# iitmdinesh/image2text

Hardware: AMD Instinct MI355X
Metric: train images/sec + greedy captions/sec, nano config (higher is better)
Workload: dtype bf16; 1 GPU; nano-224 (6x512 ViT encoder + 12x768 nanoGPT decoder, 224x224x3 images, 64-token captions); global_batch=3072, per_gpu_batch=3072, caption_len=64, parallelism=dp1, optimizer=AdamW lr 6e-4 betas (0.9,0.95), weights=random init (reference distributions)

## Files before the change

### image2text_amd/csrc/gemm.hip

```cpp
#include "common.h"
#include <stdlib.h>
#include <string.h>
#include <utility>

namespace {

constexpr int BM = 128, BN = 128, BK = 64;
constexpr int R_ROW_BYTES = 128;
constexpr int CF_ROW_BYTES = 288;
constexpr int OPERAND_BYTES = 128 * 128;
constexpr int STAGE_BYTES = 2 * OPERAND_BYTES;
constexpr int SMEM_BYTES = 2 * STAGE_BYTES;

struct GemmParams {
    const bf16_t* A;
    const bf16_t* B;
    void* C;
    int M, N, K;
    int lda, ldb, ldc;
    float alpha;
    const float* alpha_sumsq;
    const float* bias;
    int act;
    const bf16_t* aux_in;
// ... 2 lines not shown
    int ld_aux_out;
    const float* residual;
    int ldr;
    int c_is_f32;
    int accumulate;
    int tiles_m, tiles_n;
    int drop_mode;
    unsigned drop_key, drop_thr;
    float drop_scale;
    float* ws;
    int g2_splits, g2_nk;
    int g2_gn;
    int g2_dbg;
    const float* scale_a = nullptr;
    const float* scale_b = nullptr;
    int g2_stagger, g2_stagger_groups;
    const bf16_t* xq; long xq_bs; int xq_rs;
    const int* xcu;
    bf16_t* xo; long xo_bs; int xo_rs;
    float* xlse;
    int x_total_q, x_TqMax, x_H, x_d, x_B;
};

constexpr int GN_MAX = 16;
__device__ __forceinline__ void tile_coords(const GemmParams& p, int swz, int& tile_m, int& tile_n, int gn_max = GN_MAX) {
    const int gn = p.tiles_n < gn_max ? p.tiles_n : gn_max;
    const int per_group = p.tiles_m * gn;
    int grp = swz / per_group;
    const int ngroups = (p.tiles_n + gn - 1) / gn;
    int rem = swz - grp * per_group, width = gn;
// ... 816 lines not shown

#ifndef G2_SETPRIO
#define G2_SETPRIO 0
#endif
constexpr int G2_UNIT = 128 * 128;
constexpr int G2_SMEM = 8 * G2_UNIT + 8 * 4096;
typedef __attribute__((address_space(3))) void* lds_ptr_t;

struct G2Tile {
    const bf16_t* a;
    const bf16_t* b;
    unsigned a_bytes, b_bytes;
    int m0, n0, t0;
};

template <bool A_KMAJOR, bool B_KMAJOR, bool UNSWAP = false, bool XA = false>
struct G2 {
    static constexpr bool PK = A_KMAJOR && B_KMAJOR;
    static constexpr int FA = A_KMAJOR ? 2 : 1, FB = B_KMAJOR ? 2 : 1;
    static constexpr int cap(int n) { return n > 15 ? 15 : n; }
    static constexpr int LG0 = cap(4 * FA + 4 * FB), LG1 = cap(4 * FA), LG2 = cap(4 * FA), LG3 = cap(4 * FA + 4 * FB);

    static constexpr int phys(int slot) { return ((slot & 3) == 0 || (slot & 3) == 3) ? (slot >> 2) * 2 + ((slot & 3) == 3) : 4 + (slot >> 2) * 2 + ((slot & 3) == 2); }
    unsigned char* smem;
    int lane, wr, wc, wave_off, nk, tb, ta;
    int va[2][2], vb[2][2];
    unsigned step_a, step_b;
    unsigned lds0;
    G2Tile cur, nxt;

    __device__ __forceinline__ static G2Tile tile_desc(const GemmParams& p, int idx, int ntiles) {
        G2Tile d;
        if (idx >= ntiles) {
            d.a = p.A; d.b = p.B; d.a_bytes = 0; d.b_bytes = 0; d.m0 = 0; d.n0 = 0; d.t0 = 0;
            return d;
        }
        const int tiles = p.tiles_m * p.tiles_n, slice = idx / tiles;
        d.t0 = slice * p.g2_nk;
        int tile_m, tile_n;
        tile_coords(p, idx - slice * tiles, tile_m, tile_n, p.g2_gn);
        d.m0 = tile_m * 256; d.n0 = tile_n * 256;
        if (XA) {
            d.a = p.A + (size_t)tile_m * 128 * p.lda;
            d.a_bytes = (unsigned)((p.x_d + 128) * p.lda * 2);
// ... 109 lines not shown
#pragma unroll
                for (int j = 0; j < 2; ++j) rb[ks * 2 + j] = dma_frag_read<B_KMAJOR, PK>(smem + phys(SLOT) * G2_UNIT, wc * 32 + j * 16, ks, lane);
        }
    }
    template <int SUBA, int SUBB, int KS>
    __device__ __forceinline__ void mma(f32x4 (&acc)[8][4], const bf16x8 (&ra)[8], const bf16x8 (&rb)[4]) {
        if (G2_SETPRIO) __builtin_amdgcn_s_setprio(1);
#pragma unroll
        for (int i = 0; i < 4; ++i)
#pragma unroll
            for (int j = 0; j < 2; ++j)
                acc[SUBA * 4 + i][SUBB * 2 + j] =
                    (UNSWAP || (XA && SUBA == 0)) ? __builtin_amdgcn_mfma_f32_16x16x32_bf16(ra[KS * 4 + i], rb[KS * 2 + j], acc[SUBA * 4 + i][SUBB * 2 + j], 0, 0, 0)
                           : __builtin_amdgcn_mfma_f32_16x16x32_bf16(rb[KS * 2 + j], ra[KS * 4 + i], acc[SUBA * 4 + i][SUBB * 2 + j], 0, 0, 0);
        if (G2_SETPRIO) __builtin_amdgcn_s_setprio(0);
    }
    template <int LG>
    __device__ __forceinline__ void fence() {
        asm volatile("s_waitcnt vmcnt(6) lgkmcnt(%0)" ::"n"(LG) : "memory");
        __builtin_amdgcn_s_barrier();
    }

    template <bool LAST>
    __device__ __forceinline__ void two_tiles(int t, f32x4 (&acc)[8][4], bf16x8 (&ra)[8], bf16x8 (&rb0)[4], bf16x8 (&rb1)[4]) {
        fence<LG3>();  read_a<0, 1>(ra);  read_b<2>(rb1);  stage<1, 2>(t + 1);
        mma<0, 0, 0>(acc, ra, rb0);  mma<0, 0, 1>(acc, ra, rb0);
        fence<LG0>();  stage<1, 3>(t + 1);
        mma<0, 1, 0>(acc, ra, rb1);  read_a<3, 0>(ra);  mma<0, 1, 1>(acc, ra, rb1);
        fence<LG1>();  read_a<3, 1>(ra);  stage<0, 0>(t + 2);
        mma<1, 1, 0>(acc, ra, rb1);  mma<1, 1, 1>(acc, ra, rb1);
        fence<LG2>();  read_b<5>(rb1);  stage<0, 1>(t + 2);
        mma<1, 0, 0>(acc, ra, rb0);  read_a<4, 0>(ra);  mma<1, 0, 1>(acc, ra, rb0);
        fence<LG3>();  read_a<4, 1>(ra);  read_b<6>(rb0);  stage<0, 2>(t + 2);
        mma<0, 1, 0>(acc, ra, rb1);  mma<0, 1, 1>(acc, ra, rb1);
        fence<LG0>();  stage<0, 3>(t + 2);
        mma<0, 0, 0>(acc, ra, rb0);  read_a<7, 0>(ra);  mma<0, 0, 1>(acc, ra, rb0);
        fence<LG1>();  read_a<7, 1>(ra);  stage<1, 0>(t + 3);
        mma<1, 0, 0>(acc, ra, rb0);  mma<1, 0, 1>(acc, ra, rb0);
        fence<LG2>();  if (!LAST) read_b<1>(rb0);  stage<1, 1>(t + 3);
        mma<1, 1, 0>(acc, ra, rb1);  if (!LAST) read_a<0, 0>(ra);  mma<1, 1, 1>(acc, ra, rb1);
    }
    __device__ __forceinline__ void next_tile_reads(bf16x8 (&ra)[8], bf16x8 (&rb0)[4]) {
        read_b<1>(rb0);
        read_a<0, 0>(ra);
    }

    typedef __attribute__((ext_vector_type(8))) int i32x8;
// ... 102 lines not shown
    return (const GemmParams*)k;
}

template <bool A_KMAJOR, bool B_KMAJOR, int EPI>
__global__ __launch_bounds__(512) void gemm256_kernel(GemmParams p) {
    __shared__ __attribute__((aligned(16))) unsigned char smem[G2_SMEM];
    const int tid = threadIdx.x;
    const int G = gridDim.x, bid = blockIdx.x, ntiles = p.tiles_m * p.tiles_n * p.g2_splits;
    const int xcd = bid & 7, q8 = G >> 3, r8 = G & 7;
    const int first = (xcd < r8 ? xcd * (q8 + 1) : r8 * (q8 + 1) + (xcd - r8) * q8) + (bid >> 3);

    if (p.g2_stagger > 0) {
        const int k = ((bid >> 3) % p.g2_stagger_groups) * p.g2_stagger;
        for (int i = 0; i < k; ++i) __builtin_amdgcn_s_sleep(127);
    }
    G2<A_KMAJOR, B_KMAJOR, EPI == 6, EPI == 8> g;
    g.init(p, smem, tid);
    g.cur = g.tile_desc(p, first, ntiles);
    g.nxt = g.tile_desc(p, first + G, ntiles);
    f32x4 acc[8][4];
    if constexpr (EPI == 9) {
        typename decltype(g)::i32x8 fa[4], fb0[2], fb1[2];
        g.template stage<0, 0>(0); g.template stage<0, 1>(0); g.template stage<0, 2>(0); g.template stage<0, 3>(0);
        g.template stage<1, 0>(1); g.template stage<1, 1>(1);
        asm volatile("s_waitcnt vmcnt(8)" ::: "memory");
        __builtin_amdgcn_s_barrier();
        g.next_tile_reads_fp8(fa, fb0);
        for (int idx = first; idx < ntiles; idx += G) {
#pragma unroll
            for (int i = 0; i < 8; ++i)
#pragma unroll
// ... 18 lines not shown
    }
    bf16x8 ra[8], rb0[4], rb1[4];

    g.template stage<0, 0>(0); g.template stage<0, 1>(0); g.template stage<0, 2>(0); g.template stage<0, 3>(0);
    g.template stage<1, 0>(1); g.template stage<1, 1>(1);
    asm volatile("s_waitcnt vmcnt(8)" ::: "memory");
    __builtin_amdgcn_s_barrier();
    g.template read_b<1>(rb0);
    g.template read_a<0, 0>(ra);

    for (int idx = first; idx < ntiles; idx += G) {
#pragma unroll
        for (int i = 0; i < 8; ++i)
#pragma unroll
            for (int j = 0; j < 4; ++j) acc[i][j] = f32x4{0.f, 0.f, 0.f, 0.f};
        for (int t = 0; t < g.nk - 2; t += 2) g.template two_tiles<false>(t, acc, ra, rb0, rb1);
        g.template two_tiles<true>(g.nk - 2, acc, ra, rb0, rb1);
        const int m0 = g.cur.m0, n0 = g.cur.n0;
        g.cur = g.nxt;
        g.nxt = g.tile_desc(p, idx + 2 * G, ntiles);
        if constexpr (EPI == 8) {
            int lane_e = tid & 63;
            asm volatile("" : "+v"(lane_e));
            xattn_epilogue(*epilogue_params(), acc, m0 >> 8, n0, g.wr, g.wc, lane_e, smem + 8 * G2_UNIT + (g.wave_off << 2));
        } else if constexpr (EPI == 12) {
            int lane_e = tid & 63;
            asm volatile("" : "+v"(lane_e));
            top2_epilogue(*epilogue_params(), acc, m0 + g.wr * 128, n0 + g.wc * 64, lane_e);
        } else if constexpr (EPI == 6) {
            int lane_e = tid & 63;
            asm volatile("" : "+v"(lane_e));
            float* C = reinterpret_cast<float*>(p.C);
            const float alpha = eff_alpha(p);
            const int mb = m0 + g.wr * 128 + 4 * (lane_e >> 4), n_ = n0 + g.wc * 64 + (lane_e & 15);
#pragma unroll
            for (int i = 0; i < 8; ++i)
#pragma unroll
                for (int j = 0; j < 4; ++j)
#pragma unroll
                    for (int r = 0; r < 4; ++r) {
                        const int m = mb + i * 16 + r, n = n_ + j * 16;
                        if (m < p.M && n < p.N && !(p.g2_dbg & 2)) atomicAdd(C + (size_t)m * p.ldc + n, acc[i][j][r] * alpha);
                    }
        } else {
            int lane_e = tid & 63;
            asm volatile("" : "+v"(lane_e));
            const GemmParams& pe = *epilogue_params();
            const int inside = (EPI != 0 && pe.g2_dbg == 0) ?
                __builtin_amdgcn_readfirstlane((m0 + g.wr * 128 + 128 <= pe.M && n0 + g.wc * 64 + 64 <= pe.N) ? 1 : 0) : 0;
            if (pe.g2_dbg & 2) {
                if (acc[0][0][0] == 12345.678f) reinterpret_cast<float*>(pe.C)[0] = acc[7][3][3];
            } else if (inside) {
                epilogue_tile_tr<8, EPI, true>(pe, acc, m0 + g.wr * 128, n0 + g.wc * 64, lane_e, smem + 8 * G2_UNIT + (g.wave_off << 2));
            } else {
                epilogue_tile_tr<8, EPI, false>(pe, acc, m0 + g.wr * 128, n0 + g.wc * 64, lane_e, smem + 8 * G2_UNIT + (g.wave_off << 2));
            }
        }
        g.init_lane(p, tid);
// ... 355 lines not shown
    memset(&p, 0, sizeof(p));
    p.A = (const bf16_t*)A8; p.B = (const bf16_t*)B8; p.C = C;
    p.M = M; p.N = N; p.K = K / 2; p.lda = lda / 2; p.ldb = ldb / 2; p.ldc = ldc;
    p.alpha = 1.0f; p.bias = bias; p.act = act; p.residual = residual; p.ldr = ldr; p.c_is_f32 = c_is_f32;
    p.scale_a = sa; p.scale_b = sb;
    p.g2_gn = 8;
    const int n_cu = g256_cus();
    p.tiles_m = (M + 255) / 256; p.tiles_n = (N + 255) / 256;
    p.g2_splits = 1; p.g2_nk = p.K >> 6;
    const int tiles = p.tiles_m * p.tiles_n;
    hipLaunchKernelGGL((gemm256_kernel<false, false, 9>), dim3(tiles < n_cu ? tiles : n_cu), dim3(512), 0, s, p);
    return true;
}
namespace {

bool launch_g256_dw(hipStream_t s, GemmParams p) {
    const int n_cu = g256_cus();
    p.tiles_m = (p.M + 255) / 256; p.tiles_n = (p.N + 255) / 256;
    const int tiles = p.tiles_m * p.tiles_n, nk_all = (p.K + 63) >> 6;
    if (tiles >= n_cu || n_cu / tiles < 2 || i2t_det()) {
        if (g256_epilogue_class(p) != 5) return false;
        p.g2_splits = 1; p.g2_nk = (nk_all + 1) & ~1;
        hipLaunchKernelGGL((gemm256_kernel<true, true, 5>), dim3(tiles < n_cu ? tiles : n_cu), dim3(512), 0, s, p);
        return true;
    }
    int splits = n_cu / tiles;
    if (const char* e = getenv("I2T_DW_SPLITS")) splits = atoi(e);
    int per = ((nk_all + splits - 1) / splits + 1) & ~1;
    if (per < 8) per = 8;
    splits = (nk_all + per - 1) / per;
    if (splits < 2) return false;
    p.g2_splits = splits; p.g2_nk = per;
    const int items = tiles * splits;
    hipLaunchKernelGGL((gemm256_kernel<true, true, 6>), dim3(items < n_cu ? items : n_cu), dim3(512), 0, s, p);
    return true;
}

__global__ __launch_bounds__(256) void colsum_kernel(const bf16_t* __restrict__ X, int ld, int M, int N,
                                                     float* __restrict__ out, const float* __restrict__ alpha_sumsq) {
    __shared__ float part[4][512];
    const int lane = threadIdx.x & 63, w = threadIdx.x >> 6;
    const int c0 = blockIdx.x * 512 + lane * 8;
    const int rows_per = (M + gridDim.y - 1) / gridDim.y;
    const int r0 = blockIdx.y * rows_per, r1 = min(M, r0 + rows_per);
    float acc[8];
#pragma unroll
    for (int e = 0; e < 8; ++e) acc[e] = 0.f;
    if (c0 + 8 <= N) {
        int m = r0 + w;
// ... 16 lines not shown
                acc[2 * e] += bf16lo(v[e]);
                acc[2 * e + 1] += bf16hi(v[e]);
            }
        }
    } else if (c0 < N) {
        for (int m = r0 + w; m < r1; m += 4)
            for (int e = 0; e < 8 && c0 + e < N; ++e) acc[e] += bf16_to_f32(X[(size_t)m * ld + c0 + e]);
    }
#pragma unroll
    for (int e = 0; e < 8; ++e) part[w][lane * 8 + e] = acc[e];
    __syncthreads();
    for (int c = threadIdx.x; c < 512; c += 256) {
        const int n = blockIdx.x * 512 + c;
        if (n < N) atomicAdd(out + n, (part[0][c] + part[1][c] + part[2][c] + part[3][c]) * (alpha_sumsq ? 1.0f / (sqrtf(*alpha_sumsq) + 1e-6f) : 1.0f));
    }
}

template <int MT>
__global__ __launch_bounds__(256) void gemm_skinny_kernel(GemmParams p) {
    __shared__ __attribute__((aligned(16))) float red[4][MT][64][4];
    const int tid = threadIdx.x, lane = tid & 63, w = tid >> 6;
    const int g = lane >> 4, li = lane & 15;
    const int n0 = blockIdx.x * 16;
    const int nsteps_all = (p.K + 63) / 64;
    const int per = (nsteps_all + (int)gridDim.y - 1) / (int)gridDim.y;
    const int s0 = (int)blockIdx.y * per, s1 = min(nsteps_all, s0 + per);
    f32x4 acc[MT];
#pragma unroll
    for (int t = 0; t < MT; ++t) acc[t] = f32x4{0.f, 0.f, 0.f, 0.f};
    const int nrow = n0 + li;
// ... 72 lines not shown
    dim3 grid((p.N + 15) / 16, ksplit);
    hipLaunchKernelGGL(gemm_skinny_kernel<MT>, grid, dim3(256), 0, s, p);
}

}

extern "C" int i2t_gemm_bf16(void* stream, const void* A, int lda, int a_kmajor, const void* B, int ldb,
                             int b_kmajor, void* C, int ldc, int c_is_f32, int M, int N, int K, float alpha,
                             const float* bias, int act, const void* aux_in, int ld_aux_in, void* aux_out,
                             int ld_aux_out, const float* residual, int ldr, int accumulate, int drop_mode,
                             unsigned drop_key, unsigned drop_thr, float drop_scale) {
    return i2t_gemm_bf16_ex(stream, A, lda, a_kmajor, B, ldb, b_kmajor, C, ldc, c_is_f32, M, N, K, alpha, bias, act, aux_in, ld_aux_in, aux_out,
                            ld_aux_out, residual, ldr, accumulate, drop_mode, drop_key, drop_thr, drop_scale, nullptr);
}

extern "C" int i2t_gemm_bf16_ex(void* stream, const void* A, int lda, int a_kmajor, const void* B, int ldb,
                                int b_kmajor, void* C, int ldc, int c_is_f32, int M, int N, int K, float alpha,
                                const float* bias, int act, const void* aux_in, int ld_aux_in, void* aux_out,
                                int ld_aux_out, const float* residual, int ldr, int accumulate, int drop_mode,
                                unsigned drop_key, unsigned drop_thr, float drop_scale, const float* alpha_sumsq) {
    I2T_REQUIRE(A && B && C, "i2t_gemm_bf16: null operand");
    I2T_REQUIRE(M > 0 && N > 0 && K > 0, "i2t_gemm_bf16: empty problem M=%d N=%d K=%d", M, N, K);
    I2T_REQUIRE((lda & 7) == 0 && (ldb & 7) == 0, "i2t_gemm_bf16: lda=%d ldb=%d must be multiples of 8", lda, ldb);
    I2T_REQUIRE(ALIGNED16(A) && ALIGNED16(B), "i2t_gemm_bf16: A/B must be 16-byte aligned");
    I2T_REQUIRE(lda >= (a_kmajor ? ((M + 7) & ~7) : ((K + 7) & ~7)), "i2t_gemm_bf16: lda=%d too small", lda);
    I2T_REQUIRE(ldb >= (b_kmajor ? ((N + 7) & ~7) : ((K + 7) & ~7)), "i2t_gemm_bf16: ldb=%d too small", ldb);
    I2T_REQUIRE(ldc >= N, "i2t_gemm_bf16: ldc=%d < N=%d", ldc, N);
    I2T_REQUIRE(!accumulate || c_is_f32, "i2t_gemm_bf16: accumulate needs an f32 C");
    I2T_REQUIRE((act != I2T_ACT_DGELU && act != I2T_ACT_DGELU_ERF && act != I2T_ACT_MUL_AUX) || aux_in, "i2t_gemm_bf16: DGELU / MUL_AUX need aux_in");
    I2T_REQUIRE(act >= I2T_ACT_NONE && act <= I2T_ACT_MUL_AUX, "i2t_gemm_bf16: unknown act %d", act);
    I2T_REQUIRE(((uintptr_t)C & (c_is_f32 ? 15 : 7)) == 0, "i2t_gemm_bf16: C misaligned");
    GemmParams p;
    p.A = (const bf16_t*)A; p.B = (const bf16_t*)B; p.C = C;
    p.M = M; p.N = N; p.K = K; p.lda = lda; p.ldb = ldb; p.ldc = ldc;
    p.alpha = alpha; p.alpha_sumsq = alpha_sumsq; p.bias = bias; p.act = act;
// ... 19 lines not shown
    if (M <= 64 && !a_kmajor && !b_kmajor && !aux_out && act <= I2T_ACT_GELU && !accumulate && !drop_mode) {
        int ksplit = 1;
        const int ntiles = (N + 15) / 16;
        if (getenv("I2T_SKINNY_KSPLIT") && c_is_f32 && residual == (const float*)C && ldr == ldc && act == I2T_ACT_NONE && !accumulate)
            while (ntiles * ksplit < 256 && (K / 64) / (ksplit * 2) >= 2 && ksplit < 16) ksplit *= 2;
        const int mt = (M + 15) / 16;
        if (mt == 1) launch_skinny<1>(s, p, ksplit);
        else if (mt == 2) launch_skinny<2>(s, p, ksplit);
        else if (mt == 3) launch_skinny<3>(s, p, ksplit);
        else launch_skinny<4>(s, p, ksplit);
        I2T_CHECK_LAUNCH("i2t_gemm_bf16(skinny)");
        return I2T_OK;
    }
    static const char* sel = getenv("I2T_GEMM");
    static const bool no_g256 = sel && !strcmp(sel, "v1");
    if (!no_g256 && a_kmajor && b_kmajor && accumulate && c_is_f32 && !bias && act == I2T_ACT_NONE && !aux_out && !residual &&
        !drop_mode && M >= 256 && N >= 256 && (ldc & 3) == 0 && (N & 3) == 0) {
        const size_t ld_max = (size_t)(lda > ldb ? lda : ldb);
        const long k_fit = (long)((1ull << 32) / (2 * ld_max)) - 512;
        if (k_fit >= 1024) {
            const long kc = (K <= k_fit) ? K : (k_fit / 128) * 128;
            bool ok = true;
            for (long k0 = 0; k0 < K && ok; k0 += kc) {
                GemmParams q = p;
                q.A = p.A + (size_t)k0 * lda;
                q.B = p.B + (size_t)k0 * ldb;
                q.K = (int)((K - k0 < kc) ? (K - k0) : kc);
                ok = launch_g256_dw(s, q);
                if (!ok && k0 > 0) { i2t_set_error("i2t_gemm_bf16: K chunk %ld of a chunked dW GEMM has no large-tile form", k0); return I2T_EINVAL; }
            }
            if (ok) {
                I2T_CHECK_LAUNCH("i2t_gemm_bf16(256 dW)");
                return I2T_OK;
            }
        }
    }
    dim3 grid(p.tiles_m * p.tiles_n), block(256);
    int splits = 1;
    const int plain_epilogue = !bias && act == I2T_ACT_NONE && !aux_out && !residual && !drop_mode;
    if (accumulate && c_is_f32 && plain_epilogue) {
        const int tiles = p.tiles_m * p.tiles_n, nk_all = (K + BK - 1) / BK;
        while (tiles * splits < 384 && nk_all / (splits * 2) >= 4 && splits < 64) splits *= 2;
        if (i2t_det()) splits = 1;
    }
    const bool g256_ok = (K % 128 == 0 || b_kmajor) && (!a_kmajor || (size_t)(K + 512) * lda * 2 < (1ull << 32)) &&
                         (!b_kmajor || (size_t)(K + 512) * ldb * 2 < (1ull << 32));
    const char* mt_env = getenv("I2T_G256_MIN_TILES");
    const long min_tiles = mt_env ? atol(mt_env) : 40;
    {
        const char* e3 = getenv("I2T_GEMM3");
        const int g3 = e3 ? atoi(e3) : 0;
// ... 120 lines not shown

extern "C" int i2t_gemm_reserved_cus(void) { return __atomic_load_n(&g_cu_reserve, __ATOMIC_RELAXED); }

extern "C" int i2t_colsum_bf16(void* stream, const void* X, int ld, int M, int N, float* out, int accumulate) {
    return i2t_colsum_bf16_ex(stream, X, ld, M, N, out, accumulate, nullptr);
}

extern "C" int i2t_colsum_bf16_ex(void* stream, const void* X, int ld, int M, int N, float* out, int accumulate, const float* alpha_sumsq) {
    I2T_REQUIRE(X && out && M > 0 && N > 0, "i2t_colsum_bf16: bad args");
    I2T_REQUIRE((ld & 7) == 0 && ALIGNED16(X), "i2t_colsum_bf16: X must be 16-byte aligned with ld %% 8 == 0");
    hipStream_t s = (hipStream_t)stream;
    if (!accumulate) {
        hipError_t e = hipMemsetAsync(out, 0, sizeof(float) * (size_t)N, s);
        if (e != hipSuccess) { i2t_set_error("i2t_colsum_bf16: memset: %s", hipGetErrorString(e)); return I2T_EHIP; }
    }
    const int col_blocks = (N + 511) / 512;
    int splits = (M + 63) / 64;
    const int want = 512 / col_blocks;
    if (splits > want) splits = want;
    if (splits < 1 || i2t_det()) splits = 1;
    hipLaunchKernelGGL(colsum_kernel, dim3(col_blocks, splits), dim3(256), 0, s, (const bf16_t*)X, ld, M, N, out, alpha_sumsq);
    I2T_CHECK_LAUNCH("i2t_colsum_bf16");
    return I2T_OK;
}
```

### image2text_amd/engine.py

```python
import os
import re
import weakref
from types import SimpleNamespace
from typing import Dict, List, Optional, Tuple

import numpy as np
import torch

from . import ops, rng
from .engine_family import FamilyBlocks, family_spec
from .engine_llama import LlamaBlocks
from .engine_lora import LPAD, LoraAdapters
from .engine_vit import ViTEncoder
from .lib import I2TError

BF16, F32 = torch.bfloat16, torch.float32
GELU_KEEPS_DERIVATIVE = os.environ.get('I2T_GELU_DOUT', '1') != '0'
_BLOCK_SITES = {'attn_c_attn': ('attn.c_attn.weight', 'attn.c_attn.bias'), 'xattn_c_attn': ('cross_attn.in_proj_weight', 'cross_attn.in_proj_bias'),
                'mlp_c_fc': ('mlp.c_fc.weight', 'mlp.c_fc.bias'), 'mlp_c_proj': ('mlp.c_proj.weight', 'mlp.c_proj.bias')}
NORMALISER_FOLDED = os.environ.get('I2T_FOLD_NORMALISER', '1') != '0'
EMB_DROP_FUSED = os.environ.get('I2T_EMB_DROP_FUSED', '1') not in ('', '0')


VOCAB_PAD = max(8, int(os.environ.get('I2T_VOCAB_PAD', '64')) // 8 * 8)
# ... 446 lines not shown
        ops.layernorm_bwd(dln2, sv.x2, a.P(f'{pfx}.ln_2.weight'), sv.m2, sv.r2, dx, a.Gt(f'{pfx}.ln_2.weight'),
                          a.Gt(f'{pfx}.ln_2.bias'), M, d, dx_accumulate=True, dx_bf16=dxb,
                          bf16_drop=dr.get('xresid') if sv.cross else dr['resid'],
                          dx_pre_sumsq=dx_pre)
        if sv.cross:
            win = a.W(f'{pfx}.cross_attn.in_proj_weight')
            gin, gbin = a.G(f'{pfx}.cross_attn.in_proj_weight'), a.G(f'{pfx}.cross_attn.in_proj_bias')
            dco = self._empty(M, d, dtype=BF16)
            self._linear_bwd(dxb, M, d, d, sv.co, f'{pfx}.cross_attn.out_proj.weight', f'{pfx}.cross_attn.out_proj.bias',
                             dx_out=dco)
            dq, dkv = self._empty(M, d, dtype=BF16), self._empty(B, S, 2 * d, dtype=BF16)
            ops.attention_bwd(v3(sv.q, d), sv.kv[..., :d], sv.kv[..., d:], v3(sv.co, d), v3(dco, d), sv.lse_c, ws, v3(dq, d),
                              dkv[..., :d], dkv[..., d:], B, H, T, S, False, drop=dr['xattn'], cu_q=cu, total_q=M)
            dqf, dkvf = dq, dkv.view(B * S, 2 * d)
            train_in, train_inb = a.trainable(f'{pfx}.cross_attn.in_proj_weight'), a.trainable(f'{pfx}.cross_attn.in_proj_bias')
            if train_inb:
                ops.colsum(dqf, gbin[:d], M, d, accumulate=True)
            if train_in:
                ops.gemm(dqf, sv.ln3, gin[:d], d, d, M, a_kmajor=True, b_kmajor=True, accumulate=True)
            ops.gemm(dqf, win[:d], dln, M, d, d, b_kmajor=True)
            dmem32 = self._site_bwd(self._block_site(pfx, sv.layer, 'xattn_c_attn', 2 * d, d, rows=(d, 3 * d)), svlo.get('xattn_c_attn'), dkvf, sv.mem,
                                    B * S, ldrop.get('xattn_c_attn'), dx_out=dmem, accumulate=True)
            if dmem32 is not dmem:
                ops.add_(dmem, dmem32)
            ops.layernorm_bwd(dln, sv.x1, a.P(f'{pfx}.ln_3.weight'), sv.m3, sv.r3, dx, a.Gt(f'{pfx}.ln_3.weight'),
                              a.Gt(f'{pfx}.ln_3.bias'), M, d, dx_accumulate=True, dx_bf16=dxb, bf16_drop=dr['resid'])
        dao = self._empty(M, d, dtype=BF16)
        self._linear_bwd(dxb, M, d, d, sv.ao, f'{pfx}.attn.c_proj.weight',
                         f'{pfx}.attn.c_proj.bias' if a.G(f'{pfx}.attn.c_proj.bias') is not None else None, dx_out=dao)
        dqkv = self._empty(M, 3 * d, dtype=BF16)
        q3, g3 = v3(sv.qkv, 3 * d), v3(dqkv, 3 * d)
        ops.attention_bwd(q3[..., :d], q3[..., d:2 * d], q3[..., 2 * d:], v3(sv.ao, d), v3(dao, d), sv.lse, ws, g3[..., :d],
                          g3[..., d:2 * d], g3[..., 2 * d:], B, H, T, T, causal, drop=dr['sdpa'], cu_q=cu, cu_k=cu, total_q=M,
                          out_drop=dr['qkv'])
# ... 469 lines not shown
```

### image2text_amd/engine_lora.py

```python
from types import SimpleNamespace

import torch

from . import ops

BF16, F32 = torch.bfloat16, torch.float32
LPAD = 128


def _f8pad(k: int) -> int:
    return (k + 255) // 256 * 256


def fuse_guard(fp8_fuse: bool, d: int = 0, ff: int = 0) -> bool:
    return bool(fp8_fuse) and d <= 8192 and ff <= 12288


def linear_path(adapter: bool, trainable: bool, switch, fp8: bool, fp8_vit: bool, fuse: bool = False):
    e4m3 = not trainable and {'fp8': fp8, 'fp8_vit': fp8_vit, None: False}[switch]
    path = ('lora_fp8' if e4m3 else 'lora') if adapter else ('fp8' if e4m3 else 'bf16')
    return path, ('bf16' if not (e4m3 and fuse) else 'both' if adapter else 'e4m3')


class LoraAdapters:
# ... 66 lines not shown
            ops.gemm_fp8(x8, sx, e.w8, e.sw, tgt, M, s.N, _f8pad(s.K), bias=s.b, **ep)
            ops.gelu_fwd(tgt, out, erf=(act == ops.ACT_GELU_ERF))
        else:
            ops.gemm_fp8(x8, sx, e.w8, e.sw, out, M, s.N, _f8pad(s.K), bias=s.b, **ep)
        return None

    def _site_bwd(self, s, sv_l, dY, x_bf, M: int, drop_l=None, dq=None, dx_out=None, dy_sumsq=None, act=0, aux_in=None, **dx_kw):
        a, N, K = self.arena, s.N, s.K
        gW = s.G if all(a.trainable(n) for n in s.names) else None
        gb = s.gb if s.gb is not None and all(a.trainable(n) for n in s.bnames) else None
        e4m3 = self._site_e4m3(s)
        if s.lora is not None:
            assert act in (0, ops.ACT_DGELU, ops.ACT_DGELU_ERF), act
            dx32 = self._lora_bwd(s, sv_l, dY, x_bf, gW, gb, M, drop_l, e4m3, dq)
        else:
            if gb is not None:
                ops.colsum(dY, gb, M, N, accumulate=True, alpha_sumsq=dy_sumsq)
            if gW is not None:
                ops.gemm(dY, x_bf, gW, N, K, M, a_kmajor=True, b_kmajor=True, accumulate=True, alpha_sumsq=dy_sumsq)
            if dx_out is None:
                return None
            if not e4m3:
                return ops.gemm(dY, s.W, dx_out, M, K, N, b_kmajor=True, alpha_sumsq=dy_sumsq, act=act, aux_in=aux_in, **dx_kw)
            assert act in (0, ops.ACT_DGELU, ops.ACT_DGELU_ERF), act
            dx32 = self._empty(M, K) if act else dx_out
            e = self._fp8_weight(s)
            d8, sd = dq if dq is not None else self._fp8_rows(dY, M, N)
            ops.gemm_fp8(d8, sd, e.wt8, e.swt, dx32, M, K, _f8pad(N), **dx_kw)
        return ops.dgelu_mul(dx32, aux_in, dx_out, erf=(act == ops.ACT_DGELU_ERF)) if act else dx32

    def _lora_site(self, l: int, site: str):
        lo = getattr(self.dec, 'lora', None)
        if lo is None or site not in lo.sites:
            return None
# ... 52 lines not shown
        self._rank_gemm(xd if xd is not None else x, ls.A, u, M, K)
        panel = self._lora_panel(ls)
        e = self._fp8_weight(st)
        x8, sx = xq if xq is not None else self._fp8_rows(x, M, K)
        if out.dtype == F32:
            ops.gemm_fp8(x8, sx, e.w8, e.sw, out, M, N, x8.shape[1], bias=bias, residual=residual)
            ops.gemm(u, panel, out, M, N, LPAD, residual=out)
        else:
            tmp = torch.empty(M, N, dtype=F32, device=x.device)
            ops.gemm(u, panel, tmp, M, N, LPAD, residual=residual)
            ops.gemm_fp8(x8, sx, e.w8, e.sw, out, M, N, x8.shape[1], bias=bias, residual=tmp)
        return SimpleNamespace(u=u, sB=panel, xd=xd) if save else None

    def _lora_bwd(self, st, sv_l, dY, x, gW, gb, M: int, drop_l, e4m3: bool = False, dq=None):
        ls, W, K, N = st.lora, st.W, st.K, st.N
        if gb is not None:
            ops.colsum(dY, gb, M, N, accumulate=True)
        if gW is not None:
            ops.gemm(dY, x, gW, N, K, M, a_kmajor=True, b_kmajor=True, accumulate=True)
        tmp = torch.zeros(N, LPAD, dtype=F32, device=dY.device)
        ops.gemm(dY, sv_l.u, tmp, N, LPAD, M, a_kmajor=True, b_kmajor=True, accumulate=True)
        for row0, nrows, col0, B, GB in ls.parts:
            GB.add_(tmp[row0:row0 + nrows, col0:col0 + B.shape[1]], alpha=ls.scale)
        du = torch.empty(M, LPAD, dtype=BF16, device=dY.device)
        self._rank_gemm(dY, sv_l.sB, du, M, N, b_kmajor=True)
        xd = sv_l.xd if sv_l.xd is not None else x
        ops.gemm(du, xd, ls.GA, LPAD, K, M, a_kmajor=True, b_kmajor=True, accumulate=True)
        dx = torch.empty(M, K, dtype=F32, device=dY.device)
        if e4m3:
            e = self._fp8_weight(st)
            d8, sd = dq if dq is not None else self._fp8_rows(dY, M, N)
            ops.gemm_fp8(d8, sd, e.wt8, e.swt, dx, M, K, d8.shape[1])
        else:
            ops.gemm(dY, W, dx, M, K, N, b_kmajor=True)
# ... 39 lines not shown
```

### image2text_amd/lib.py

```python
import ctypes as C
import os

import torch

_HERE = os.path.dirname(os.path.abspath(__file__))
LIB_PATH = os.environ.get('I2T_LIB') or os.path.join(_HERE, 'csrc', 'libi2t_hip.so')

P, I, L, F, I64, U = C.c_void_p, C.c_int, C.c_long, C.c_float, C.c_int64, C.c_uint

SIGNATURES = {
    'i2t_abi_version': [],
    'i2t_last_error': [C.c_char_p, C.c_size_t],
    'i2t_gemm_bf16': [P, P, I, I, P, I, I, P, I, I, I, I, I, F, P, I, P, I, P, I, P, I, I, I, U, U, F],
    'i2t_gemm_bf16_ex': [P, P, I, I, P, I, I, P, I, I, I, I, I, F, P, I, P, I, P, I, P, I, I, I, U, U, F, P],
    'i2t_gemm_reserve_cus': [I],
    'i2t_gemm_reserved_cus': [],
    'i2t_xattn_kv_fused': [P, P, I, P, I, P, P, L, I, P, I, P, I, P, L, I, P, I, I, I, I, U, U, F],
    'i2t_colsum_bf16': [P, P, I, I, I, P, I],
    'i2t_colsum_bf16_ex': [P, P, I, I, I, P, I, P],
    'i2t_layernorm_fwd': [P, P, P, P, P, I, P, P, I, I],
    'i2t_layernorm_fwd_eps': [P, P, P, P, P, I, P, P, I, I, F],
    'i2t_layernorm_bwd': [P, P, I, P, P, P, P, P, I, P, P, P, I, I, U, U, F, P, P],
    'i2t_layernorm_bwd_ex': [P, P, I, P, P, P, P, P, I, P, P, P, I, I, U, U, F, P, P, U, U, F, I, I],
    'i2t_layernorm_nd_fwd': [P, P, P, P, P, P, L, P, I, I, I],
    'i2t_layernorm_nd_fwd_drop': [P, P, P, P, P, P, L, P, I, I, I, U, U, F, L],
    'i2t_layernorm_nd_bwd': [P, P, L, P, P, P, P, P, P, P, P, I, I, I],
    'i2t_attention_fwd': [P, P, L, I, P, L, I, P, L, I, P, L, I, P, I, I, I, I, I, U, U, F, P, P, I],
    'i2t_attention_bwd': [P, P, L, I, P, L, I, P, L, I, P, L, I, P, L, I, P, P, P, L, I, P, L, I, P, L, I, I, I, I, I, I, U, U, F, P, P, I, U, U, F],
    'i2t_attention_bwd_ex': [P, P, L, I, P, L, I, P, L, I, P, L, I, P, L, I, P, P, P, L, I, P, L, I, P, L, I, I, I, I, I, I, U, U, F, P, P, I, U, U, F, I],
    'i2t_embed_fwd': [P, P, P, P, P, I, I, I, I, I, P],
    'i2t_embed_bwd': [P, P, P, P, P, I, I, I, I, I, P],
    'i2t_ce_fwd': [P, P, I, P, P, F, I64, P, P, I, I],
    'i2t_ce_bwd': [P, P, I, P, P, F, I64, P, P, I, I],
    'i2t_ce_fwd_bwd': [P, P, I, P, P, F, I64, P, P, I, I],
# ... 133 lines not shown
```

### image2text_amd/ops.py

```python
import os
import weakref
from typing import Optional

import torch

from . import lib as _l

BF16 = torch.bfloat16
F32 = torch.float32


def _lib():
    return _l.load()


def _stream() -> int:
    return torch.cuda.current_stream().cuda_stream


def _p(t: Optional[torch.Tensor]):
    return None if t is None else t.data_ptr()


def _need_cuda(*ts):
# ... 61 lines not shown
        _gemm(a, b_lo, acc, M, N, K, lda=lda, ldb=ldb, ldc=ldacc, accumulate=True, **kw)
        n += 1
    PRECISE_CALLS['gemm'] += 1
    PRECISE_CALLS['products'] += n
    if not direct:
        if out.dtype == F32:
            raise _l.I2TError('I2T_PRECISE=1: an activated GEMM writes bf16 operands')
        lo = torch.empty_like(out)
        split_f32(acc, out, lo, act=act)
        out._i2t_lo = lo
    return out


def gemm(a: torch.Tensor, b: torch.Tensor, out: torch.Tensor, M: int, N: int, K: int, *, a_kmajor=False, b_kmajor=False,
         lda=None, ldb=None, ldc=None, alpha=1.0, bias=None, act=0, aux_in=None, aux_out=None, residual=None,
         ldr=None, accumulate=False, drop=None, workspace=None, alpha_sumsq=None):
    if precise():
        return _gemm_precise(a, b, out, M, N, K, a_kmajor=a_kmajor, b_kmajor=b_kmajor, lda=lda, ldb=ldb, ldc=ldc, alpha=alpha, bias=bias,
                             act=act, aux_in=aux_in, aux_out=aux_out, residual=residual, ldr=ldr, accumulate=accumulate, drop=drop,
                             alpha_sumsq=alpha_sumsq)
    return _gemm(a, b, out, M, N, K, a_kmajor=a_kmajor, b_kmajor=b_kmajor, lda=lda, ldb=ldb, ldc=ldc, alpha=alpha, bias=bias, act=act,
                 aux_in=aux_in, aux_out=aux_out, residual=residual, ldr=ldr, accumulate=accumulate, drop=drop, workspace=workspace,
                 alpha_sumsq=alpha_sumsq)


def _gemm(a, b, out, M, N, K, *, a_kmajor=False, b_kmajor=False, lda=None, ldb=None, ldc=None, alpha=1.0, bias=None, act=0, aux_in=None,
          aux_out=None, residual=None, ldr=None, accumulate=False, drop=None, workspace=None, alpha_sumsq=None):
    _need_cuda(a, b, out)
    assert a.dtype == BF16 and b.dtype == BF16 and out.dtype in (BF16, F32)
    lda = a.stride(0) if lda is None else lda
    ldb = b.stride(0) if ldb is None else ldb
# ... 29 lines not shown
def gemm_reserve_cus(n: int):
    _l.check(_lib().i2t_gemm_reserve_cus(int(n)), 'i2t_gemm_reserve_cus')


def gemm_reserved_cus() -> int:
    return int(_lib().i2t_gemm_reserved_cus())


def colsum(x: torch.Tensor, out: torch.Tensor, M: int, N: int, ld=None, accumulate=False, alpha_sumsq=None):
    _need_cuda(x, out)
    _l.check(_lib().i2t_colsum_bf16_ex(_stream(), _p(x), x.stride(0) if ld is None else ld, M, N, _p(out), int(accumulate), _p(alpha_sumsq)),
             'i2t_colsum_bf16_ex')
    return out


def layernorm_fwd(x, gamma, beta, y, mean, rstd, M, d, eps=None):
    _need_cuda(x, y)
    if y.dtype == BF16 and precise():
        y32 = torch.empty(y.shape, dtype=F32, device=y.device)
        layernorm_fwd(x, gamma, beta, y32, mean, rstd, M, d, eps)
        y._i2t_lo = torch.empty_like(y)
        return split_f32(y32, y, y._i2t_lo)
    if eps is not None:
        _l.check(_lib().i2t_layernorm_fwd_eps(_stream(), _p(x), _p(gamma), _p(beta), _p(y), int(y.dtype == F32), _p(mean), _p(rstd),
                                              M, d, float(eps)), 'i2t_layernorm_fwd_eps')
        return y
    _l.check(_lib().i2t_layernorm_fwd(_stream(), _p(x), _p(gamma), _p(beta), _p(y), int(y.dtype == F32), _p(mean), _p(rstd),
                                      M, d), 'i2t_layernorm_fwd')
    return y

# ... 674 lines not shown
```

### include/i2t.h

```cpp
#ifndef I2T_H
#define I2T_H
#include <stddef.h>
#include <stdint.h>

#ifdef __cplusplus
extern "C" {
#endif

#define I2T_OK 0
#define I2T_EINVAL (-1)
#define I2T_EHIP (-2)

#define I2T_ABI_VERSION 5

int i2t_abi_version(void);
int i2t_last_error(char* buf, size_t n);

#define I2T_ACT_NONE 0
#define I2T_ACT_GELU 1
#define I2T_ACT_DGELU 2
#define I2T_ACT_GELU_ERF 3
#define I2T_ACT_DGELU_ERF 4
#define I2T_ACT_GELU_DOUT 5
#define I2T_ACT_MUL_AUX 6
// ... 22 lines not shown
                     const float* alpha_sumsq);

int i2t_xattn_kv_fused(void* stream, const void* mem, int ld_mem, const void* w_kv, int ld_w, const float* bias_kv,
                       const void* q, long q_bs, int q_rs, const int* cu_q, int total_q, void* kv, int ld_kv, void* o,
                       long o_bs, int o_rs, float* lse, int B, int S, int H, int Tq, unsigned drop_key, unsigned drop_thr,
                       float drop_scale);

int i2t_gemm_bf16_ws(void* stream, const void* A, int lda, const void* B, int ldb, void* C, int ldc, int c_is_f32, int M, int N, int K,
                     const float* bias, int act, const float* residual, int ldr, float* workspace, long ws_floats);

int i2t_gemm_reserve_cus(int n_reserved);
int i2t_gemm_reserved_cus(void);

int i2t_colsum_bf16(void* stream, const void* X, int ld, int M, int N, float* out, int accumulate);
int i2t_colsum_bf16_ex(void* stream, const void* X, int ld, int M, int N, float* out, int accumulate, const float* alpha_sumsq);

int i2t_layernorm_fwd(void* stream, const float* x, const float* gamma, const float* beta,
                      void* y, int y_is_f32, float* mean, float* rstd, int M, int d);
int i2t_layernorm_fwd_eps(void* stream, const float* x, const float* gamma, const float* beta,
                          void* y, int y_is_f32, float* mean, float* rstd, int M, int d, float eps);
int i2t_layernorm_bwd(void* stream, const void* dy, int dy_is_f32, const float* x, const float* gamma,
                      const float* mean, const float* rstd,
                      float* dx, int dx_accumulate, void* dx_bf16, float* dgamma, float* dbeta, int M, int d,
                      unsigned drop_key, unsigned drop_thr, float drop_scale, float* sumsq_out, const float* dx_pre_sumsq);
int i2t_layernorm_bwd_ex(void* stream, const void* dy, int dy_is_f32, const float* x, const float* gamma,
                         const float* mean, const float* rstd,
                         float* dx, int dx_accumulate, void* dx_bf16, float* dgamma, float* dbeta, int M, int d,
                         unsigned drop_key, unsigned drop_thr, float drop_scale, float* sumsq_out, const float* dx_pre_sumsq,
                         unsigned dx_mask_key, unsigned dx_mask_thr, float dx_mask_scale, int acc_period, int acc_rows);

// ... 232 lines not shown
```

Before: 10110 images/s.

## Fold bias-gradient column sum into split-K dW GEMM via extra MFMA with ones

Adds a fused path that computes the bias gradient (column sum of dY) inside the split-K 256-tile dW GEMM kernel. It multiplies the already-loaded A fragments by a ones vector with extra MFMAs on one tile column and atomically adds the result in the epilogue. This removes the separate colsum kernel launch and its second full read of dY. The cost is extra inline-asm branches and MFMAs in the hot loop, plus more atomics. Non-split paths still launch the standalone colsum.

```diff
diff --git a/image2text_amd/csrc/gemm.hip b/image2text_amd/csrc/gemm.hip
--- a/image2text_amd/csrc/gemm.hip
+++ b/image2text_amd/csrc/gemm.hip
@@ -40,6 +40,7 @@
     int g2_dbg;
     const float* scale_a = nullptr;
     const float* scale_b = nullptr;
+    float* colsum_out = nullptr;
     int g2_stagger, g2_stagger_groups;
     const bf16_t* xq; long xq_bs; int xq_rs;
     const int* xcu;
@@ -886,7 +887,7 @@
     int m0, n0, t0;
 };
 
-template <bool A_KMAJOR, bool B_KMAJOR, bool UNSWAP = false, bool XA = false>
+template <bool A_KMAJOR, bool B_KMAJOR, bool UNSWAP = false, bool XA = false, bool CS = false>
 struct G2 {
     static constexpr bool PK = A_KMAJOR && B_KMAJOR;
     static constexpr int FA = A_KMAJOR ? 2 : 1, FB = B_KMAJOR ? 2 : 1;
@@ -900,6 +901,46 @@
     unsigned step_a, step_b;
     unsigned lds0;
     G2Tile cur, nxt;
+    f32x4 cs0, cs1;
+    int cs_c, cs_t, cs_j, cs_n;
+    u32x4 cs_ones;
+    __device__ __forceinline__ void cs_begin(const GemmParams& p, int n0) {
+        cs0 = cs1 = f32x4{0.f, 0.f, 0.f, 0.f};
+        cs_ones = u32x4{0x3f803f80u, 0x3f803f80u, 0x3f803f80u, 0x3f803f80u};
+        asm volatile("" : "+v"(cs_ones));
+        cs_c = 0; cs_j = n0 >> 8; cs_n = p.tiles_n;
+    }
+    __device__ __forceinline__ void cs_tile() {
+        cs_t = cs_c;
+        cs_c = cs_c + 1 == cs_n ? 0 : cs_c + 1;
+    }
+    template <int SUBA, int KS>
+    __device__ __forceinline__ void cs_mma(const bf16x8 (&ra)[8]) {
+        asm volatile("s_cmp_lg_u32 %[t], %[j]\n\t"
+                     "s_cbranch_scc1 .Lcs_end_%=\n\t"
+                     "s_nop 1\n\t"
+                     "s_cmp_lt_u32 %[wc], 2\n\t"
+                     "s_cbranch_scc0 .Lcs_hi_%=\n\t"
+                     "s_cmp_eq_u32 %[wc], 0\n\t"
+                     "s_cbranch_scc0 .Lcs_1_%=\n\t"
+                     "v_mfma_f32_16x16x32_bf16 %[c], %[o], %[f0], %[c]\n\t"
+                     "s_branch .Lcs_end_%=\n"
+                     ".Lcs_1_%=:\n\t"
+                     "v_mfma_f32_16x16x32_bf16 %[c], %[o], %[f1], %[c]\n\t"
+                     "s_branch .Lcs_end_%=\n"
+                     ".Lcs_hi_%=:\n\t"
+                     "s_cmp_eq_u32 %[wc], 2\n\t"
+                     "s_cbranch_scc0 .Lcs_3_%=\n\t"
+                     "v_mfma_f32_16x16x32_bf16 %[c], %[o], %[f2], %[c]\n\t"
+                     "s_branch .Lcs_end_%=\n"
+                     ".Lcs_3_%=:\n\t"
+                     "v_mfma_f32_16x16x32_bf16 %[c], %[o], %[f3], %[c]\n"
+                     ".Lcs_end_%=:"
+                     : [c] "+v"(SUBA ? cs1 : cs0)
+                     : [o] "v"(cs_ones), [f0] "v"(ra[KS * 4 + 0]), [f1] "v"(ra[KS * 4 + 1]), [f2] "v"(ra[KS * 4 + 2]), [f3] "v"(ra[KS * 4 + 3]),
+                       [t] "s"(cs_t), [j] "s"(cs_j), [wc] "s"(wc)
+                     : "scc");
+    }
 
     __device__ __forceinline__ static G2Tile tile_desc(const GemmParams& p, int idx, int ntiles) {
         G2Tile d;
@@ -1039,6 +1080,7 @@
                     (UNSWAP || (XA && SUBA == 0)) ? __builtin_amdgcn_mfma_f32_16x16x32_bf16(ra[KS * 4 + i], rb[KS * 2 + j], acc[SUBA * 4 + i][SUBB * 2 + j], 0, 0, 0)
                            : __builtin_amdgcn_mfma_f32_16x16x32_bf16(rb[KS * 2 + j], ra[KS * 4 + i], acc[SUBA * 4 + i][SUBB * 2 + j], 0, 0, 0);
         if (G2_SETPRIO) __builtin_amdgcn_s_setprio(0);
+        if constexpr (CS && KS == SUBB) cs_mma<SUBA, KS>(ra);
     }
     template <int LG>
     __device__ __forceinline__ void fence() {
@@ -1048,6 +1090,7 @@
 
     template <bool LAST>
     __device__ __forceinline__ void two_tiles(int t, f32x4 (&acc)[8][4], bf16x8 (&ra)[8], bf16x8 (&rb0)[4], bf16x8 (&rb1)[4]) {
+        if constexpr (CS) cs_tile();
         fence<LG3>();  read_a<0, 1>(ra);  read_b<2>(rb1);  stage<1, 2>(t + 1);
         mma<0, 0, 0>(acc, ra, rb0);  mma<0, 0, 1>(acc, ra, rb0);
         fence<LG0>();  stage<1, 3>(t + 1);
@@ -1056,6 +1099,7 @@
         mma<1, 1, 0>(acc, ra, rb1);  mma<1, 1, 1>(acc, ra, rb1);
         fence<LG2>();  read_b<5>(rb1);  stage<0, 1>(t + 2);
         mma<1, 0, 0>(acc, ra, rb0);  read_a<4, 0>(ra);  mma<1, 0, 1>(acc, ra, rb0);
+        if constexpr (CS) cs_tile();
         fence<LG3>();  read_a<4, 1>(ra);  read_b<6>(rb0);  stage<0, 2>(t + 2);
         mma<0, 1, 0>(acc, ra, rb1);  mma<0, 1, 1>(acc, ra, rb1);
         fence<LG0>();  stage<0, 3>(t + 2);
@@ -1188,7 +1232,7 @@
         const int k = ((bid >> 3) % p.g2_stagger_groups) * p.g2_stagger;
         for (int i = 0; i < k; ++i) __builtin_amdgcn_s_sleep(127);
     }
-    G2<A_KMAJOR, B_KMAJOR, EPI == 6, EPI == 8> g;
+    G2<A_KMAJOR, B_KMAJOR, EPI == 6 || EPI == 13, EPI == 8, EPI == 13> g;
     g.init(p, smem, tid);
     g.cur = g.tile_desc(p, first, ntiles);
     g.nxt = g.tile_desc(p, first + G, ntiles);
@@ -1237,6 +1281,7 @@
         for (int i = 0; i < 8; ++i)
 #pragma unroll
             for (int j = 0; j < 4; ++j) acc[i][j] = f32x4{0.f, 0.f, 0.f, 0.f};
+        if constexpr (EPI == 13) g.cs_begin(p, g.cur.n0);
         for (int t = 0; t < g.nk - 2; t += 2) g.template two_tiles<false>(t, acc, ra, rb0, rb1);
         g.template two_tiles<true>(g.nk - 2, acc, ra, rb0, rb1);
         const int m0 = g.cur.m0, n0 = g.cur.n0;
@@ -1250,7 +1295,7 @@
             int lane_e = tid & 63;
             asm volatile("" : "+v"(lane_e));
             top2_epilogue(*epilogue_params(), acc, m0 + g.wr * 128, n0 + g.wc * 64, lane_e);
-        } else if constexpr (EPI == 6) {
+        } else if constexpr (EPI == 6 || EPI == 13) {
             int lane_e = tid & 63;
             asm volatile("" : "+v"(lane_e));
             float* C = reinterpret_cast<float*>(p.C);
@@ -1265,6 +1310,13 @@
                         const int m = mb + i * 16 + r, n = n_ + j * 16;
                         if (m < p.M && n < p.N && !(p.g2_dbg & 2)) atomicAdd(C + (size_t)m * p.ldc + n, acc[i][j][r] * alpha);
                     }
+            if constexpr (EPI == 13) {
+                asm volatile("s_nop 15\n\ts_nop 15\n\ts_nop 15" : "+v"(g.cs0), "+v"(g.cs1));
+                const float norm = p.alpha_sumsq ? 1.0f / (sqrtf(*p.alpha_sumsq) + 1e-6f) : 1.0f;
+                const int m = m0 + g.wr * 128 + g.wc * 16 + lane_e;
+                if (lane_e < 16 && m < p.M) atomicAdd(p.colsum_out + m, g.cs0[0] * norm);
+                if (lane_e < 16 && m + 64 < p.M) atomicAdd(p.colsum_out + m + 64, g.cs1[0] * norm);
+            }
         } else {
             int lane_e = tid & 63;
             asm volatile("" : "+v"(lane_e));
@@ -1650,13 +1702,16 @@
 }
 namespace {
 
-bool launch_g256_dw(hipStream_t s, GemmParams p) {
+void launch_colsum(hipStream_t s, const bf16_t* X, int ld, int M, int N, float* out, const float* alpha_sumsq);
+
+bool launch_g256_dw(hipStream_t s, GemmParams p, bool fold_colsum = true) {
     const int n_cu = g256_cus();
     p.tiles_m = (p.M + 255) / 256; p.tiles_n = (p.N + 255) / 256;
     const int tiles = p.tiles_m * p.tiles_n, nk_all = (p.K + 63) >> 6;
     if (tiles >= n_cu || n_cu / tiles < 2 || i2t_det()) {
         if (g256_epilogue_class(p) != 5) return false;
         p.g2_splits = 1; p.g2_nk = (nk_all + 1) & ~1;
+        if (p.colsum_out) launch_colsum(s, p.A, p.lda, p.K, p.M, p.colsum_out, p.alpha_sumsq);
         hipLaunchKernelGGL((gemm256_kernel<true, true, 5>), dim3(tiles < n_cu ? tiles : n_cu), dim3(512), 0, s, p);
         return true;
     }
@@ -1668,7 +1723,12 @@
     if (splits < 2) return false;
     p.g2_splits = splits; p.g2_nk = per;
     const int items = tiles * splits;
-    hipLaunchKernelGGL((gemm256_kernel<true, true, 6>), dim3(items < n_cu ? items : n_cu), dim3(512), 0, s, p);
+    if (p.colsum_out && !fold_colsum) {
+        launch_colsum(s, p.A, p.lda, p.K, p.M, p.colsum_out, p.alpha_sumsq);
+        p.colsum_out = nullptr;
+    }
+    if (p.colsum_out) hipLaunchKernelGGL((gemm256_kernel<true, true, 13>), dim3(items < n_cu ? items : n_cu), dim3(512), 0, s, p);
+    else hipLaunchKernelGGL((gemm256_kernel<true, true, 6>), dim3(items < n_cu ? items : n_cu), dim3(512), 0, s, p);
     return true;
 }
 
@@ -1715,6 +1775,15 @@
         const int n = blockIdx.x * 512 + c;
         if (n < N) atomicAdd(out + n, (part[0][c] + part[1][c] + part[2][c] + part[3][c]) * (alpha_sumsq ? 1.0f / (sqrtf(*alpha_sumsq) + 1e-6f) : 1.0f));
     }
+}
+
+void launch_colsum(hipStream_t s, const bf16_t* X, int ld, int M, int N, float* out, const float* alpha_sumsq) {
+    const int col_blocks = (N + 511) / 512;
+    int splits = (M + 63) / 64;
+    const int want = 512 / col_blocks;
+    if (splits > want) splits = want;
+    if (splits < 1 || i2t_det()) splits = 1;
+    hipLaunchKernelGGL(colsum_kernel, dim3(col_blocks, splits), dim3(256), 0, s, X, ld, M, N, out, alpha_sumsq);
 }
 
 template <int MT>
@@ -1817,11 +1886,33 @@
                             ld_aux_out, residual, ldr, accumulate, drop_mode, drop_key, drop_thr, drop_scale, nullptr);
 }
 
+static int gemm_bf16_impl(void* stream, const void* A, int lda, int a_kmajor, const void* B, int ldb,
+                          int b_kmajor, void* C, int ldc, int c_is_f32, int M, int N, int K, float alpha,
+                          const float* bias, int act, const void* aux_in, int ld_aux_in, void* aux_out,
+                          int ld_aux_out, const float* residual, int ldr, int accumulate, int drop_mode,
+                          unsigned drop_key, unsigned drop_thr, float drop_scale, const float* alpha_sumsq, float* colsum_out);
+
 extern "C" int i2t_gemm_bf16_ex(void* stream, const void* A, int lda, int a_kmajor, const void* B, int ldb,
                                 int b_kmajor, void* C, int ldc, int c_is_f32, int M, int N, int K, float alpha,
                                 const float* bias, int act, const void* aux_in, int ld_aux_in, void* aux_out,
                                 int ld_aux_out, const float* residual, int ldr, int accumulate, int drop_mode,
                                 unsigned drop_key, unsigned drop_thr, float drop_scale, const float* alpha_sumsq) {
+    return gemm_bf16_impl(stream, A, lda, a_kmajor, B, ldb, b_kmajor, C, ldc, c_is_f32, M, N, K, alpha, bias, act, aux_in, ld_aux_in, aux_out,
+                          ld_aux_out, residual, ldr, accumulate, drop_mode, drop_key, drop_thr, drop_scale, alpha_sumsq, nullptr);
+}
+
+extern "C" int i2t_gemm_dw_colsum_bf16(void* stream, const void* A, int lda, const void* B, int ldb, float* C, int ldc, int M, int N, int K,
+                                       float alpha, const float* alpha_sumsq, float* colsum_out) {
+    I2T_REQUIRE(((uintptr_t)colsum_out & 3) == 0, "i2t_gemm_dw_colsum_bf16: colsum_out misaligned");
+    return gemm_bf16_impl(stream, A, lda, 1, B, ldb, 1, C, ldc, 1, M, N, K, alpha, nullptr, I2T_ACT_NONE, nullptr, 0, nullptr, 0, nullptr, 0, 1, 0,
+                          0u, 0u, 1.0f, alpha_sumsq, colsum_out);
+}
+
+static int gemm_bf16_impl(void* stream, const void* A, int lda, int a_kmajor, const void* B, int ldb,
+                          int b_kmajor, void* C, int ldc, int c_is_f32, int M, int N, int K, float alpha,
+                          const float* bias, int act, const void* aux_in, int ld_aux_in, void* aux_out,
+                          int ld_aux_out, const float* residual, int ldr, int accumulate, int drop_mode,
+                          unsigned drop_key, unsigned drop_thr, float drop_scale, const float* alpha_sumsq, float* colsum_out) {
     I2T_REQUIRE(A && B && C, "i2t_gemm_bf16: null operand");
     I2T_REQUIRE(M > 0 && N > 0 && K > 0, "i2t_gemm_bf16: empty problem M=%d N=%d K=%d", M, N, K);
     I2T_REQUIRE((lda & 7) == 0 && (ldb & 7) == 0, "i2t_gemm_bf16: lda=%d ldb=%d must be multiples of 8", lda, ldb);
@@ -1871,6 +1962,8 @@
     }
     static const char* sel = getenv("I2T_GEMM");
     static const bool no_g256 = sel && !strcmp(sel, "v1");
+    const char* fold_env = getenv("I2T_FOLD_COLSUM");
+    const bool fold_colsum = !(fold_env && fold_env[0] == '0');
     if (!no_g256 && a_kmajor && b_kmajor && accumulate && c_is_f32 && !bias && act == I2T_ACT_NONE && !aux_out && !residual &&
         !drop_mode && M >= 256 && N >= 256 && (ldc & 3) == 0 && (N & 3) == 0) {
         const size_t ld_max = (size_t)(lda > ldb ? lda : ldb);
@@ -1883,7 +1976,8 @@
                 q.A = p.A + (size_t)k0 * lda;
                 q.B = p.B + (size_t)k0 * ldb;
                 q.K = (int)((K - k0 < kc) ? (K - k0) : kc);
-                ok = launch_g256_dw(s, q);
+                q.colsum_out = colsum_out;
+                ok = launch_g256_dw(s, q, fold_colsum);
                 if (!ok && k0 > 0) { i2t_set_error("i2t_gemm_bf16: K chunk %ld of a chunked dW GEMM has no large-tile form", k0); return I2T_EINVAL; }
             }
             if (ok) {
@@ -1892,6 +1986,7 @@
             }
         }
     }
+    if (colsum_out) launch_colsum(s, p.A, lda, K, M, colsum_out, alpha_sumsq);
     dim3 grid(p.tiles_m * p.tiles_n), block(256);
     int splits = 1;
     const int plain_epilogue = !bias && act == I2T_ACT_NONE && !aux_out && !residual && !drop_mode;
@@ -2042,12 +2137,7 @@
         hipError_t e = hipMemsetAsync(out, 0, sizeof(float) * (size_t)N, s);
         if (e != hipSuccess) { i2t_set_error("i2t_colsum_bf16: memset: %s", hipGetErrorString(e)); return I2T_EHIP; }
     }
-    const int col_blocks = (N + 511) / 512;
-    int splits = (M + 63) / 64;
-    const int want = 512 / col_blocks;
-    if (splits > want) splits = want;
-    if (splits < 1 || i2t_det()) splits = 1;
-    hipLaunchKernelGGL(colsum_kernel, dim3(col_blocks, splits), dim3(256), 0, s, (const bf16_t*)X, ld, M, N, out, alpha_sumsq);
+    launch_colsum(s, (const bf16_t*)X, ld, M, N, out, alpha_sumsq);
     I2T_CHECK_LAUNCH("i2t_colsum_bf16");
     return I2T_OK;
 }
diff --git a/image2text_amd/engine.py b/image2text_amd/engine.py
--- a/image2text_amd/engine.py
+++ b/image2text_amd/engine.py
@@ -484,10 +484,10 @@
                               dkv[..., :d], dkv[..., d:], B, H, T, S, False, drop=dr['xattn'], cu_q=cu, total_q=M)
             dqf, dkvf = dq, dkv.view(B * S, 2 * d)
             train_in, train_inb = a.trainable(f'{pfx}.cross_attn.in_proj_weight'), a.trainable(f'{pfx}.cross_attn.in_proj_bias')
-            if train_inb:
+            if train_in:
+                ops.gemm(dqf, sv.ln3, gin[:d], d, d, M, a_kmajor=True, b_kmajor=True, accumulate=True, colsum_out=gbin[:d] if train_inb else None)
+            elif train_inb:
                 ops.colsum(dqf, gbin[:d], M, d, accumulate=True)
-            if train_in:
-                ops.gemm(dqf, sv.ln3, gin[:d], d, d, M, a_kmajor=True, b_kmajor=True, accumulate=True)
             ops.gemm(dqf, win[:d], dln, M, d, d, b_kmajor=True)
             dmem32 = self._site_bwd(self._block_site(pfx, sv.layer, 'xattn_c_attn', 2 * d, d, rows=(d, 3 * d)), svlo.get('xattn_c_attn'), dkvf, sv.mem,
                                     B * S, ldrop.get('xattn_c_attn'), dx_out=dmem, accumulate=True)
diff --git a/image2text_amd/engine_lora.py b/image2text_amd/engine_lora.py
--- a/image2text_amd/engine_lora.py
+++ b/image2text_amd/engine_lora.py
@@ -104,10 +104,10 @@
             assert act in (0, ops.ACT_DGELU, ops.ACT_DGELU_ERF), act
             dx32 = self._lora_bwd(s, sv_l, dY, x_bf, gW, gb, M, drop_l, e4m3, dq)
         else:
-            if gb is not None:
+            if gW is not None:
+                ops.gemm(dY, x_bf, gW, N, K, M, a_kmajor=True, b_kmajor=True, accumulate=True, alpha_sumsq=dy_sumsq, colsum_out=gb)
+            elif gb is not None:
                 ops.colsum(dY, gb, M, N, accumulate=True, alpha_sumsq=dy_sumsq)
-            if gW is not None:
-                ops.gemm(dY, x_bf, gW, N, K, M, a_kmajor=True, b_kmajor=True, accumulate=True, alpha_sumsq=dy_sumsq)
             if dx_out is None:
                 return None
             if not e4m3:
@@ -190,10 +190,10 @@
 
     def _lora_bwd(self, st, sv_l, dY, x, gW, gb, M: int, drop_l, e4m3: bool = False, dq=None):
         ls, W, K, N = st.lora, st.W, st.K, st.N
-        if gb is not None:
+        if gW is not None:
+            ops.gemm(dY, x, gW, N, K, M, a_kmajor=True, b_kmajor=True, accumulate=True, colsum_out=gb)
+        elif gb is not None:
             ops.colsum(dY, gb, M, N, accumulate=True)
-        if gW is not None:
-            ops.gemm(dY, x, gW, N, K, M, a_kmajor=True, b_kmajor=True, accumulate=True)
         tmp = torch.zeros(N, LPAD, dtype=F32, device=dY.device)
         ops.gemm(dY, sv_l.u, tmp, N, LPAD, M, a_kmajor=True, b_kmajor=True, accumulate=True)
         for row0, nrows, col0, B, GB in ls.parts:
diff --git a/image2text_amd/lib.py b/image2text_amd/lib.py
--- a/image2text_amd/lib.py
+++ b/image2text_amd/lib.py
@@ -18,6 +18,7 @@
     'i2t_xattn_kv_fused': [P, P, I, P, I, P, P, L, I, P, I, P, I, P, L, I, P, I, I, I, I, U, U, F],
     'i2t_colsum_bf16': [P, P, I, I, I, P, I],
     'i2t_colsum_bf16_ex': [P, P, I, I, I, P, I, P],
+    'i2t_gemm_dw_colsum_bf16': [P, P, I, P, I, P, I, I, I, I, F, P, P],
     'i2t_layernorm_fwd': [P, P, P, P, P, I, P, P, I, I],
     'i2t_layernorm_fwd_eps': [P, P, P, P, P, I, P, P, I, I, F],
     'i2t_layernorm_bwd': [P, P, I, P, P, P, P, P, I, P, P, P, I, I, U, U, F, P, P],
diff --git a/image2text_amd/ops.py b/image2text_amd/ops.py
--- a/image2text_amd/ops.py
+++ b/image2text_amd/ops.py
@@ -99,7 +99,10 @@
 
 def gemm(a: torch.Tensor, b: torch.Tensor, out: torch.Tensor, M: int, N: int, K: int, *, a_kmajor=False, b_kmajor=False,
          lda=None, ldb=None, ldc=None, alpha=1.0, bias=None, act=0, aux_in=None, aux_out=None, residual=None,
-         ldr=None, accumulate=False, drop=None, workspace=None, alpha_sumsq=None):
+         ldr=None, accumulate=False, drop=None, workspace=None, alpha_sumsq=None, colsum_out=None):
+    if colsum_out is not None:
+        assert a_kmajor and b_kmajor and accumulate and bias is None and not act and aux_out is None and residual is None and drop is None
+        return gemm_dw_colsum(a, b, out, colsum_out, M, N, K, alpha=alpha, alpha_sumsq=alpha_sumsq, lda=lda, ldb=ldb, ldc=ldc)
     if precise():
         return _gemm_precise(a, b, out, M, N, K, a_kmajor=a_kmajor, b_kmajor=b_kmajor, lda=lda, ldb=ldb, ldc=ldc, alpha=alpha, bias=bias,
                              act=act, aux_in=aux_in, aux_out=aux_out, residual=residual, ldr=ldr, accumulate=accumulate, drop=drop,
@@ -159,6 +162,20 @@
     return out
 
 
+def gemm_dw_colsum(dy: torch.Tensor, x: torch.Tensor, gw: torch.Tensor, gb, N: int, K: int, M: int, *, alpha=1.0, alpha_sumsq=None,
+                   lda=None, ldb=None, ldc=None):
+    if precise():
+        if gb is not None:
+            colsum(dy, gb, M, N, ld=lda, accumulate=True, alpha_sumsq=alpha_sumsq)
+        return gemm(dy, x, gw, N, K, M, a_kmajor=True, b_kmajor=True, lda=lda, ldb=ldb, ldc=ldc, alpha=alpha, accumulate=True, alpha_sumsq=alpha_sumsq)
+    _need_cuda(dy, x, gw)
+    assert dy.dtype == BF16 and x.dtype == BF16 and gw.dtype == F32 and (gb is None or gb.dtype == F32)
+    _l.check(_lib().i2t_gemm_dw_colsum_bf16(_stream(), _p(dy), dy.stride(0) if lda is None else lda, _p(x), x.stride(0) if ldb is None else ldb,
+                                            _p(gw), gw.stride(0) if ldc is None else ldc, N, K, M, float(alpha), _p(alpha_sumsq), _p(gb)),
+             'i2t_gemm_dw_colsum_bf16')
+    return gw
+
+
 def layernorm_fwd(x, gamma, beta, y, mean, rstd, M, d, eps=None):
     _need_cuda(x, y)
     if y.dtype == BF16 and precise():
diff --git a/include/i2t.h b/include/i2t.h
--- a/include/i2t.h
+++ b/include/i2t.h
@@ -60,6 +60,8 @@
 
 int i2t_colsum_bf16(void* stream, const void* X, int ld, int M, int N, float* out, int accumulate);
 int i2t_colsum_bf16_ex(void* stream, const void* X, int ld, int M, int N, float* out, int accumulate, const float* alpha_sumsq);
+int i2t_gemm_dw_colsum_bf16(void* stream, const void* A, int lda, const void* B, int ldb, float* C, int ldc, int M, int N, int K,
+                            float alpha, const float* alpha_sumsq, float* colsum_out);
 
 int i2t_layernorm_fwd(void* stream, const float* x, const float* gamma, const float* beta,
                       void* y, int y_is_f32, float* mean, float* rstd, int M, int d);
```

Measured after the change: 10230 images/s (median of 6 runs). 1.01x the previous value.
